# epam/ai-dial-rag

Hardware: AMD Instinct MI355X
Metric: retrieval_qps_10Mx384 (higher is better)
Workload: dtype f32 (int8 MFMA filter with exact integer dot products and a rigorous error margin, every candidate the margin cannot exclude re-scored in f64 with the reference formula)

## Files before the change

ai-dial-rag_amd/csrc/vec_index.hip:

```cpp
#include <algorithm>
#include <cmath>
#include <cstdarg>
#include <cstdio>
#include <cstdlib>
#include <cstring>
#include <mutex>
#include <new>
#include <type_traits>
#include <vector>

#include "common.h"
#include "vec_kernels.h"
#include "vec_kernels_f16.h"
#include "vec_kernels_q16.h"
#include "vec_kernels_h16.h"
#include "vec_kernels_sieve.h"
#include "vec_kernels_i8.h"
#include "vec_kernels_exact.h"
#include "vec_kernels_scoped.h"

namespace mir {

static thread_local char g_err[512] = "";

// ... 174 lines not shown
static void launch_row_norms(const T *src, int64_t n, int d, mir_index *ix, hipStream_t stream) {
    unsigned int *mx = reinterpret_cast<unsigned int *>(ix->d_maxnorm);
    const int rows_per_wg = std::min<int64_t>(128, kNormsLdsBytes / ((int64_t)norms_row_stride(d) * 4));
    if (rows_per_wg >= 32) {
        const size_t lds = (size_t)rows_per_wg * norms_row_stride(d) * 4;
        row_norms_lds_kernel<T><<<dim3((unsigned)((n + rows_per_wg - 1) / rows_per_wg)), dim3(256), lds, stream>>>(
            src, n, d, rows_per_wg, ix->d_docsq, ix->d_invnorm, mx);
    } else {
        row_norms_kernel<T><<<dim3((unsigned)((n + 255) / 256)), dim3(256), 0, stream>>>(src, n, d, ix->d_docsq, ix->d_invnorm, mx);
    }
}

static int32_t build_derived(mir_index *ix, hipStream_t stream) {
    const int64_t n = ix->n;
    const int d = ix->d;
    ix->ksteps = ix->native16 ? (d + 511) / 512 * 32 : pad_ksteps(d);
    ix->layout16 = !ix->native16 && (ix->ksteps == 8 || ix->ksteps == 16 || ix->ksteps == 24);
    ix->n_tiles = (uint32_t)((n + kTileRows - 1) / kTileRows);
    ix->hi_only = ix->layout16 && sieve_sized(ix);
    ix->wide16 = wide64_split(ix) && sieve_sized(ix);
    ix->ks16 = ix->wide16 ? (d + 511) / 512 * 32 : 0;
    const size_t split_bytes = ix->wide16 ? 16 : (size_t)ix->n_tiles * ix->ksteps * ((ix->native16 || ix->hi_only) ? 1024 : 2048);
    const size_t aux_bytes = (size_t)(ix->n_tiles + 1) * kTileRows * sizeof(float);
    MIR_HIP(hipMalloc(&ix->d_split, std::max<size_t>(split_bytes, 16)));
    MIR_HIP(hipMalloc(&ix->d_docsq, std::max<size_t>(aux_bytes, 16)));
    MIR_HIP(hipMalloc(&ix->d_invnorm, std::max<size_t>(aux_bytes, 16)));
    MIR_HIP(hipMalloc(&ix->d_maxnorm, 32));
    MIR_HIP(hipMalloc(&ix->d_dnorm, std::max<size_t>((size_t)n * 4, 16)));
    ix->hbm_bytes += split_bytes + 2 * aux_bytes + 32 + (size_t)n * 4;
    MIR_HIP(hipMemsetAsync(ix->d_docsq, 0, std::max<size_t>(aux_bytes, 16), stream));
    MIR_HIP(hipMemsetAsync(ix->d_invnorm, 0, std::max<size_t>(aux_bytes, 16), stream));
    MIR_HIP(hipMemsetAsync(ix->d_maxnorm, 0, 32, stream));
    MIR_HIP(hipMemsetAsync(reinterpret_cast<char *>(ix->d_maxnorm) + 16, 0xff, 4, stream));
    MIR_HIP(hipMalloc(reinterpret_cast<void **>(&ix->d_stats), 64));
    MIR_HIP(hipMemsetAsync(ix->d_stats, 0, 64, stream));
    if (n > 0) {
        const int64_t total_lanes = (int64_t)ix->n_tiles * ix->ksteps * 64;
        const int64_t blocks = (total_lanes + 255) / 256;
        MIR_REQUIRE(blocks < (int64_t)0x7fffffff, "index too large for one pack launch");
        if (ix->native16) {
            pack_f16_16_kernel<<<dim3((unsigned)blocks), dim3(256), 0, stream>>>(ix->d_f16, n, d, ix->ksteps / 2, total_lanes,
                                                                               ix->d_split);
            MIR_HIP(hipGetLastError());
            launch_row_norms(ix->d_f16, n, d, ix, stream);
        } else if (ix->layout16) {
            const int64_t lanes16 = total_lanes;
            pack_split16_f32_kernel<<<dim3((unsigned)((lanes16 + 255) / 256)), dim3(256), 0, stream>>>(ix->d_orig, n, d, ix->ksteps / 2,
                                                                                                   lanes16, ix->d_split, ix->hi_only);
            MIR_HIP(hipGetLastError());
            launch_row_norms(ix->d_orig, n, d, ix, stream);
        } else if (ix->wide16) {
            const int64_t lanes = (int64_t)ix->n_tiles * ix->ks16 * 64;
            MIR_HIP(hipMalloc(reinterpret_cast<void **>(&ix->d_hi16), (size_t)ix->n_tiles * ix->ks16 * 1024));
            ix->hbm_bytes += (size_t)ix->n_tiles * ix->ks16 * 1024;
            pack_hi16_f32_kernel<<<dim3((unsigned)((lanes + 255) / 256)), dim3(256), 0, stream>>>(ix->d_orig, n, d, ix->ks16 / 2, lanes, ix->d_hi16);
            MIR_HIP(hipGetLastError());
            launch_row_norms(ix->d_orig, n, d, ix, stream);
        } else {
            pack_split_f32_kernel<<<dim3((unsigned)blocks), dim3(256), 0, stream>>>(ix->d_orig, n, d, ix->ksteps,
                                                                                  total_lanes, ix->d_split);
            MIR_HIP(hipGetLastError());
            launch_row_norms(ix->d_orig, n, d, ix, stream);
        }
        MIR_HIP(hipGetLastError());
        if (ix->native16) row_dnorm_kernel<_Float16><<<dim3((unsigned)((n + 3) / 4)), dim3(256), 0, stream>>>(ix->d_f16, n, d, ix->d_dnorm);
        else row_dnorm_kernel<float><<<dim3((unsigned)((n + 3) / 4)), dim3(256), 0, stream>>>(ix->d_orig, n, d, ix->d_dnorm);
        MIR_HIP(hipGetLastError());
        if (ix->layout16) {
// ... 350 lines not shown

template <int KIND>
static int32_t launch_sieve(const mir_index *ix, int qpw, const uint4 *qsplit_g, const double *q_norm_g, const double *q_sq_g,
                            const double *q_err_g, int nq, int nwg,
                            uint32_t tile0, uint32_t n_tiles, int nan_guard, const uint64_t *gthr_g, uint64_t *cand, float *candv,
                            uint32_t *ccount, float *part_sample, bool sample, unsigned long long *stat, hipStream_t stream) {
    const float *aux = scan_aux<KIND>(ix);
    const int ks32 = ix->ksteps / 2;
    const size_t lds = sieve_lds_bytes(ks32);
    const uint32_t n_rows = (uint32_t)ix->n;
#define MIR_SIEVE_PICK(KS, P)                                                                                          \
    (qpw > 128 ? (sample ? sieve_q16_kernel<KS, KIND, true, 2, P> : sieve_q16_kernel<KS, KIND, false, 2, P>)           \
               : (sample ? sieve_q16_kernel<KS, KIND, true, 1, P> : sieve_q16_kernel<KS, KIND, false, 1, P>))
    auto go = [&](auto kern) {
        return launch_dyn(kern, dim3(nwg), dim3(512), lds, stream, ix->d_split, aux, qsplit_g, q_norm_g, q_sq_g, q_err_g, ix->d_maxnorm,
                          n_rows, tile0, n_tiles, nq, nan_guard, gthr_g, cand, candv, ccount, part_sample, stat,
                          (uint32_t)(ks32 * 2 * 64), ix->d_tilemax);
    };
    switch (ks32) {
        case 4: return go(ix->norms_spread ? MIR_SIEVE_PICK(4, true) : MIR_SIEVE_PICK(4, false));
        case 8: return go(ix->norms_spread ? MIR_SIEVE_PICK(8, true) : MIR_SIEVE_PICK(8, false));
        case 12: return go(ix->norms_spread ? MIR_SIEVE_PICK(12, true) : MIR_SIEVE_PICK(12, false));
        default:
            set_error("internal: the sieve has no instance for %d k-steps of 32", ks32);
            return MIR_ERR_UNSUPPORTED;
    }
#undef MIR_SIEVE_PICK
}

template <int KIND>
static int32_t launch_sieve_i8(const mir_index *ix, int qpw, const float *q_scale_g, const uint4 *qfrag_g, const double *q_norm_g,
                               const double *q_sq_g, const double *q_err_g, int nq, int nwg, uint32_t stage0, uint32_t n_stages,
                               int nan_guard, const uint64_t *gthr_g, uint64_t *cand, float *candv, uint32_t *ccount, float *part_sample,
                               bool sample, unsigned long long *stat, hipStream_t stream) {
    const bool four = nq >= kI8FourWaveQueries;
    const size_t lds = sieve_i8_lds_bytes(ix->ks64, four ? 4 : 8);
    const uint32_t n_rows = (uint32_t)ix->n;
    const int grid = (four && !sample) ? 2 * nwg : nwg;
#define MIR_I8_PICK(KS)                                                                                                \
    (four ? (qpw > 128 ? (sample ? sieve_i8_kernel<KS, KIND, true, 4, 4> : sieve_i8_kernel<KS, KIND, false, 4, 4>)     \
                       : (sample ? sieve_i8_kernel<KS, KIND, true, 2, 4> : sieve_i8_kernel<KS, KIND, false, 2, 4>))    \
          : (qpw > 128 ? (sample ? sieve_i8_kernel<KS, KIND, true, 2, 8> : sieve_i8_kernel<KS, KIND, false, 2, 8>)     \
                       : (sample ? sieve_i8_kernel<KS, KIND, true, 1, 8> : sieve_i8_kernel<KS, KIND, false, 1, 8>)))
    auto go = [&](auto kern) {
        return launch_dyn(kern, dim3(grid), dim3(four ? 256 : 512), lds, stream, ix->d_i8,
                          ix->d_i8rec + (KIND == SCAN_COS ? (size_t)ix->n_stages * 72 : 0), qfrag_g, q_norm_g, q_sq_g, q_err_g, ix->d_i8stats,
                          q_scale_g, n_rows, stage0, n_stages, nq, nan_guard, gthr_g, cand, candv, ccount, part_sample, stat);
    };
    switch (ix->ks64) {
        case 2: return go(MIR_I8_PICK(2));
        case 4: return go(MIR_I8_PICK(4));
        case 6: return go(MIR_I8_PICK(6));
        default:
            set_error("internal: the int8 filter has no instance for %d k-steps of 64", ix->ks64);
            return MIR_ERR_UNSUPPORTED;
    }
#undef MIR_I8_PICK
}

template <int KIND, bool BF = false>
static int32_t launch_sieve16(const mir_index *ix, const uint4 *qfrag_g, const float *qscale_g, const double *q_norm_g, const double *q_sq_g,
                              int nq, int nwg, uint32_t tile0, uint32_t n_tiles, int nan_guard, const uint64_t *gthr_g, uint64_t *cand,
                              float *candv, uint32_t *ccount, float *part_sample, bool sample, unsigned long long *stat, hipStream_t stream,
                              const double *q_err_g = nullptr) {
    const float *aux = scan_aux<KIND>(ix);
    const size_t lds = sieve16_lds_bytes();
    const uint32_t n_rows = (uint32_t)ix->n;
    const uint4 *image = BF ? ix->d_hi16 : ix->d_split;
    const int ks = BF ? ix->ks16 : ix->ksteps;
    auto go = [&](auto kern) {
        return launch_dyn(kern, dim3(nwg), dim3(512), lds, stream, image, aux, qfrag_g, qscale_g, q_norm_g, q_sq_g, q_err_g, ix->d_maxnorm,
                          n_rows, tile0, n_tiles, nq, nan_guard, gthr_g, cand, candv, ccount, part_sample, stat);
    };
    if (ks == 64) return go(sample ? sieve_h16_kernel<32, KIND, true, BF> : sieve_h16_kernel<32, KIND, false, BF>);
    if (ks == 32) return go(sample ? sieve_h16_kernel<16, KIND, true, BF> : sieve_h16_kernel<16, KIND, false, BF>);
    set_error("internal: the float16 sieve has no instance for %d k-steps", ks);
    return MIR_ERR_UNSUPPORTED;
}

template <int KIND>
// ... 170 lines not shown
    } else if (ix->native16) {
        const int ks32 = ix->ksteps / 2, ntiles16 = ngroups * (kQ16Queries / 16);
        query_stats_h16_kernel<<<dim3(std::max(b, (gwords + 63) / 64)), dim3(64), 0, stream>>>(dq, b, d, sb.q_sq, sb.q_norm, sb.qscale, gz, gwords);
        prep_queries_h16_kernel<<<dim3(ntiles16 * ks32), dim3(64), 0, stream>>>(dq, b, d, ks32, sb.qscale, sb.qsplit);
    } else {
        const int ntiles32 = ngroups * (qpw / 32);
        const int prep_blocks = std::max(ntiles32 * ix->ksteps + b, (gwords + 63) / 64);
        prep_queries_kernel<<<dim3(prep_blocks), dim3(64), 0, stream>>>(dq, b, d, ix->ksteps, ntiles32, sb.qsplit, sb.q_sq, sb.q_norm, gz, gwords);
    }
    MIR_HIP(hipGetLastError());
    return MIR_OK;
}

struct SieveGroup {
    int g, q0, nq;
    int guard;
    uint64_t *gthr;
};

static int32_t sieve_filter(const SearchCall &c, const SieveGroup &sg, uint32_t t0, uint32_t nt, int wgs, uint64_t *cand, float *cv,
                            uint32_t *cc, bool smp) {
    mir_index *ix = c.ix;
    const SearchBuffers &sb = c.sb;
    const hipStream_t stream = c.stream;
    const int g = sg.g, q0 = sg.q0, nq = sg.nq, guard = sg.guard, qpw = c.pl.qpw;
    uint64_t *gt = sg.gthr;
    const double *qn = sb.q_norm + q0, *qsq = sb.q_sq + q0, *qerr = sb.q_err + q0;
    float *ps = reinterpret_cast<float *>(sb.part_sample);
    unsigned long long *st = smp ? nullptr : ix->d_stats + (t0 ? 1 : 0);
    if (c.use_i8) {
        const uint32_t s0 = t0 / 2, s1 = std::min<uint32_t>((t0 + nt + 1) / 2, ix->n_stages);
        const uint4 *qf = sb.qsplit + (size_t)g * (qpw / 16) * ix->ks64 * 64;
        return with_kind(c.metric, [&](auto kind) {
            return launch_sieve_i8<kind()>(ix, qpw, sb.qscale + q0, qf, qn, qsq, qerr, nq, wgs, s0, s1 - s0, guard, gt, cand, cv, cc, ps, smp, st, stream);
        });
    }
    if (ix->native16) {
        const uint4 *qs16 = sb.qsplit + (size_t)g * (kQ16Queries / 16) * (ix->ksteps / 2) * 64;
        const float *qsc = sb.qscale + (size_t)g * qpw;
        return with_kind(c.metric, [&](auto kind) {
            return launch_sieve16<kind()>(ix, qs16, qsc, qn, qsq, nq, wgs, t0, nt, guard, gt, cand, cv, cc, ps, smp, st, stream);
        });
    }
    if (ix->wide16) {
        const uint4 *qw = sb.qsplit + (size_t)g * (kQ16Queries / 16) * (ix->ks16 / 2) * 128;
        return with_kind(c.metric, [&](auto kind) {
            return launch_sieve16<kind(), true>(ix, qw, nullptr, qn, qsq, nq, wgs, t0, nt, guard, gt, cand, cv, cc, ps, smp, st, stream, qerr);
        });
    }
    const uint4 *qs = sb.qsplit + (size_t)g * (qpw / 32) * ix->ksteps * 128;
    return with_kind(c.metric, [&](auto kind) {
        return launch_sieve<kind()>(ix, qpw, qs, qn, qsq, qerr, nq, wgs, t0, nt, guard, gt, cand, cv, cc, ps, smp, st, stream);
    });
}

static SieveSelectArgs sieve_select_args(const SearchCall &c, const SieveGroup &sg) {
    const mir_index *ix = c.ix;
    const SearchBuffers &sb = c.sb;
    SieveSelectArgs sa;
    sa.l = sb.sv; sa.q0 = sg.q0; sa.nq = sg.nq; sa.k = c.k; sa.metric = c.metric; sa.d = ix->d; sa.nan_guard = sg.guard;
    sa.rel_err = ix->native16 ? (float)kH16RelErr : kHiHiRelErr;
    sa.extra_slop = ix->wide16 ? wide_accum_slop(ix->ks16 * 16) : 0.f;
    sa.docs = ix->d_orig; sa.docs16 = ix->d_f16; sa.doc_sq = ix->d_docsq;
    sa.dnorm = (ix->native16 || !ix->norms_spread) ? nullptr : ix->d_dnorm;
    sa.q = c.dq; sa.q_sq = sb.q_sq; sa.q_norm = sb.q_norm; sa.max_norm = ix->d_maxnorm;
    sa.q_err = ix->native16 ? nullptr : sb.q_err;
    sa.i8_qscale = nullptr;
// ... 21 lines not shown
    sg.g = g; sg.q0 = qpw * g; sg.nq = std::min(qpw, c.b - qpw * g);
    sg.guard = c.metric == MIR_METRIC_EUCLIDEAN_DIST ? 1 : 0;
    sg.gthr = sb.gthr + (size_t)g * std::max(128, qpw);
    const int nq = sg.nq;
    unsigned long long *gt = reinterpret_cast<unsigned long long *>(sg.gthr);
    SieveScatterArgs ca;
    ca.q0 = sg.q0; ca.nq = nq; ca.l = sb.sv;
    SieveSelectArgs sa = sieve_select_args(c, sg);
    int32_t rc = sieve_filter(c, sg, 0, (uint32_t)kSampleWgs * pl.sample_tpw, kSampleWgs, nullptr, nullptr, nullptr, true);
    if (rc != MIR_OK) return rc;
    if (c.use_i8) {
        SieveSampleArgs ta;
        ta.part = reinterpret_cast<const float *>(sb.part_sample); ta.nwg = kSampleWgs; ta.qpw = qpw; ta.k = k; ta.nq = nq;
        ta.q0 = sg.q0; ta.d = ix->d; ta.metric = c.metric; ta.docs = ix->d_orig; ta.doc_sq = ix->d_docsq;
        ta.q = c.dq; ta.q_sq = sb.q_sq; ta.q_norm = sb.q_norm; ta.gthr = gt;
        sieve_sample_threshold_kernel<<<dim3(nq), dim3(256), 0, stream>>>(ta);
    } else {
        sample_threshold_kernel<<<dim3(nq), dim3(256), 0, stream>>>(reinterpret_cast<const float *>(sb.part_sample), kSampleWgs, qpw, k, nq, gt);
    }
    MIR_HIP(hipGetLastError());
    ProfileBracket prof(ix, stream);
    rc = prof.begin();
    if (rc != MIR_OK) return rc;
    for (int phase = pl.tiles_first ? 0 : 1; phase < 2; ++phase) {
        const size_t region = c.use_i8 ? (size_t)kI8Region : (size_t)kSieveRegion;
        uint64_t *cand = sb.sv_cand + (size_t)phase * nwg * region;
        float *cv = sb.sv_candv + (size_t)phase * nwg * region;
        uint32_t *cc = sb.sv_ccount + (size_t)phase * nwg * (c.use_i8 ? 8 : 1);
        rc = phase == 0 ? sieve_filter(c, sg, 0, pl.tiles_first, nwg, cand, cv, cc, false)
                        : sieve_filter(c, sg, pl.tiles_first, ix->n_tiles - pl.tiles_first, nwg, cand, cv, cc, false);
        if (rc == MIR_OK && phase == 1) rc = prof.end();
        if (rc != MIR_OK) return rc;
        ca.cand = cand; ca.candv = cv; ca.ccount = cc;
        if (c.use_i8) sieve_scatter_i8_kernel<<<dim3(nwg * 8), dim3(256), 0, stream>>>(ca);
        else sieve_scatter_kernel<<<dim3(nwg * kSieveScatterSplit), dim3(256), 0, stream>>>(ca);
        sa.mode = phase;
        rc = launch_dyn(sieve_select_kernel, dim3(nq), dim3(kSieveSelectThreads), sieve_select_lds_bytes(), stream, sa);
        if (rc != MIR_OK) return rc;
    }
    return MIR_OK;
}

static int32_t enqueue_list_group(const SearchCall &c, int g) {
    const mir_index *ix = c.ix;
    const SearchBuffers &sb = c.sb;
    const hipStream_t stream = c.stream;
    const int nwg = c.pl.nwg, klist = c.pl.klist, qpw = c.pl.qpw, metric = c.metric;
    const uint4 *qs = sb.qsplit + (size_t)g * (qpw / 32) * ix->ksteps * 128;
    uint64_t *pg = sb.part + (size_t)g * nwg * qpw * klist;
    const int nq = std::min(qpw, c.b - qpw * g);
    ProfileBracket prof(c.ix, stream);
    int32_t rc = prof.begin();
    if (rc != MIR_OK) return rc;
    if (qpw == 32) {
        rc = with_kind(metric, [&](auto kind) { return launch_scan<kind()>(ix, qs, nq, klist, nwg, pg, stream); });
    } else if (ix->native16) {
        const uint4 *qs16 = sb.qsplit + (size_t)g * (kQ16Queries / 16) * (ix->ksteps / 2) * 64;
        const float *qsc = sb.qscale + (size_t)g * qpw;
        rc = with_kind(metric, [&](auto kind) { return launch_scan_h16<kind()>(ix, qs16, qsc, nq, klist, nwg, pg, sb.gthr + (size_t)g * 128, stream); });
    } else if (ix->layout16) {
        const double *qn = sb.q_norm + (size_t)g * qpw;
        rc = with_kind(metric, [&](auto kind) { return launch_scan_q16<kind()>(ix, qs, qn, nq, klist, nwg, pg, stream); });
    } else {
        rc = with_kind(metric, [&](auto kind) { return launch_scan_f16<kind()>(ix, qs, nq, klist, nwg, pg, stream); });
    }
    if (rc != MIR_OK) return rc;
    return prof.end();
}
// ... 422 lines not shown
    double ms = 0.0;
    for (auto &pr : ev) {
        float t = 0.f;
        hipError_t e = hipEventSynchronize(pr.second);
        if (e == hipSuccess) e = hipEventElapsedTime(&t, pr.first, pr.second);
        {
            std::lock_guard<std::mutex> lk(idx->mu);
            idx->prof_free.push_back(pr.first);
            idx->prof_free.push_back(pr.second);
        }
        if (e != hipSuccess) {
            set_error("profile read failed: %s", hipGetErrorString(e));
            return MIR_ERR_HIP;
        }
        ms += t;
    }
    std::lock_guard<std::mutex> lk(idx->mu);
    idx->prof_launches += (int64_t)ev.size();
    idx->prof_ms += ms;
    if (launches) *launches = idx->prof_launches;
    if (total_ms) *total_ms = idx->prof_ms;
    if (reset) {
        idx->prof_launches = 0;
        idx->prof_ms = 0.0;
    }
    return MIR_OK;
}

int32_t mir_index_scan_stats(mir_index *idx, int32_t reset, int64_t *out8) {
    MIR_REQUIRE(idx != nullptr && out8 != nullptr, "NULL argument");
    int32_t rc = use_device(idx->device, nullptr);
    if (rc != MIR_OK) return rc;
    MIR_HIP(hipDeviceSynchronize());
    MIR_HIP(hipMemcpy(out8, idx->d_stats, 64, hipMemcpyDeviceToHost));
    if (reset) MIR_HIP(hipMemset(idx->d_stats, 0, 64));
    out8[6] = idx->i8 ? 1 : 0;
    return MIR_OK;
}

int32_t mir_index_search_device(mir_index *idx, const double *queries_device, int32_t b, int32_t k,
                                int32_t metric, int32_t *out_doc, int64_t *out_chunk, int64_t *out_row,
                                double *out_dist, int32_t *out_count, int32_t *out_flags, void *stream_) {
    int32_t rc = check_search_args(idx, queries_device, b, k, metric, out_count);
    if (rc != MIR_OK) return rc;
    if (b == 0) return MIR_OK;
    rc = use_device(idx->device, nullptr);
    if (rc != MIR_OK) return rc;
    SearchPlan pl;
    rc = plan(idx, b, k, &pl);
    if (rc != MIR_OK) return rc;
    SearchBuffers sb;
    const SearchOut out{out_doc, out_chunk, out_row, out_dist, out_count, out_flags};
    return with_workspace(
        idx, static_cast<hipStream_t>(stream_), false, [&](char *base) { return carve(sb, base, idx, b, k, pl, false); },
        [&](Workspace *, hipStream_t s) { return enqueue_search(idx, queries_device, b, k, metric, sb, pl, out, s); });
}

int32_t mir_index_search(mir_index *idx, const double *queries_host, int32_t b, int32_t k, int32_t metric,
                         int32_t *out_doc, int64_t *out_chunk, int64_t *out_row, double *out_dist,
                         int32_t *out_count, int32_t *out_flags) {
    int32_t rc = check_search_args(idx, queries_host, b, k, metric, out_count);
    if (rc != MIR_OK) return rc;
    if (b == 0) return MIR_OK;
    rc = use_device(idx->device, nullptr);
    if (rc != MIR_OK) return rc;
    SearchPlan pl;
    rc = plan(idx, b, k, &pl);
    if (rc != MIR_OK) return rc;
// ... 409 lines not shown
```

ai-dial-rag_amd/csrc/vec_kernels_i8.h:

```cpp
#pragma once
#include "vec_kernels_sieve.h"

#ifndef I8_ABL
#define I8_ABL 0
#endif

namespace mir {

typedef int __attribute__((ext_vector_type(4))) i32x4;

constexpr int kI8StatWords = 8;
constexpr int kI8MaxK = 16;
static_assert(kI8MaxK <= kSieveSampleMaxK, "the exact sample threshold evaluates k rows in one round");
constexpr int kI8Region = 32768;
constexpr int kI8WavePart = kI8Region / 8;
__device__ __forceinline__ void i8_margin_ab(float qn, float eq, const float *__restrict__ stats, float &A, float &B) {
    i8_margin_ab_decl(qn, eq, stats, A, B);
}
__device__ __forceinline__ float i8_margin_tile(bool l2, float A, float B, float e_t, float s_t, float sq) {
    const float m = fmaf(e_t, A, B) + 2.0f * s_t * sq;
    return l2 ? 2.0f * m : m;
}

__global__ __launch_bounds__(256) void i8_tile_scale_kernel(const float *__restrict__ src, int64_t n, int d, float4 *__restrict__ tparam) {
// ... 137 lines not shown
        qfrag[(int64_t)blk * 64 + lane] = make_uint4(wv[0], wv[1], wv[2], wv[3]);
    } else {
        const int qi = blk - ntiles16 * ks64;
        if (qi >= b) return;
        const float m = q_amax[qi];
        const bool ok = m >= 0.f;
        const float inv = m > 0.f ? 127.0f / m : 1.0f;
        const float sq = 1.0f / inv;
        double e2 = 0.0;
        for (int j = lane; j < d; j += 64) {
            const double x = q[(int64_t)qi * d + j];
            const double r = ok ? x - (double)sq * (double)i8_quant((float)x, inv) : x;
            e2 += r * r;
        }
        e2 = wave_sum(e2);
        if (lane == 0) {
            q_err[qi] = sqrt(e2);
            q_scale[qi] = sq;
        }
    }
}

__host__ __device__ constexpr int sieve_i8_stages(int nw) { return nw == 8 ? kSieveStages : 3; }
__host__ __device__ constexpr size_t sieve_i8_lds_bytes(int ks64, int nw) { return (size_t)sieve_i8_stages(nw) * (ks64 * 4 * 1024 + (64 + 8) * 4) + 64; }

template <int KS64, int KIND, bool SAMPLE, int QT, int NW>
__global__ __launch_bounds__(NW * 64, 2) void sieve_i8_kernel(const uint4 *__restrict__ docs, const float *__restrict__ aux,
                                                          const uint4 *__restrict__ qfrag, const double *__restrict__ q_norm,
                                                          const double *__restrict__ q_sq, const double *__restrict__ q_err,
                                                          const float *__restrict__ stats, const float *__restrict__ q_scale,
                                                          uint32_t n_rows, uint32_t stage0, uint32_t n_stages, int nq, int nan_guard,
                                                          const uint64_t *__restrict__ gthr, uint64_t *__restrict__ cand,
                                                          float *__restrict__ candv, uint32_t *__restrict__ ccount,
                                                          float *__restrict__ part_sample, unsigned long long *__restrict__ stat) {
    static_assert(KIND == SCAN_L2 || KIND == SCAN_IP || KIND == SCAN_COS, "scan kind");
    static_assert(QT == 1 || QT == 2 || QT == 4, "query tiles per wave");
    static_assert(NW == 8 || NW == 4, "waves per workgroup");
    constexpr int NS = sieve_i8_stages(NW);
    constexpr int APW = 64 / NW;
    constexpr int NB = KS64 * 2;
    constexpr int SB = NB * 2;
    constexpr int STAGE_U4 = SB * 64;
    constexpr int PPW = SB / NW;
    constexpr int PW = PPW + 1;
    constexpr int AS = 64 + 8;
    constexpr int D = NS - 1;
    constexpr int QPL = NW * 16 * QT;
    static_assert(SB % NW == 0, "sieve_i8: d padded to a multiple of 128");
    extern __shared__ __attribute__((aligned(16))) unsigned char smem[];
    uint4 *ring = reinterpret_cast<uint4 *>(smem);
    float *aux_lds = reinterpret_cast<float *>(smem + (size_t)NS * STAGE_U4 * 16);

    const int tid = threadIdx.x, lane = tid & 63, qc = lane & 15, jg = lane >> 4;
    const int wave8 = __builtin_amdgcn_readfirstlane(tid >> 6);
    const uint32_t G = gridDim.x;

    const float amin = KIND == SCAN_L2 ? stats[7] : 0.f;
    int qloc[QT];
    bool lane_live[QT];
    unsigned long long live_mask[QT];
    constexpr float L = KIND == SCAN_L2 ? 2.0f : 1.0f;
    const float ax_hi = KIND == SCAN_COS ? stats[6] : 1.0f;
    float tbc[QT];
    float sq[QT], mA[QT], mB[QT], P1[QT], A1[QT], guard[QT], best[QT];
    uint32_t brow[QT];
    i32x4 qh[QT][KS64];
    const bool active = nq > wave8 * QT * 16;
// ... 189 lines not shown
            if (KS64 < QT + 1 && have_prev) {
#pragma unroll
                for (int u = KS64 - 1; u < QT; ++u) filter(u, p0[u], p1[u], pax, pt, ptp);
            }
#pragma unroll
            for (int u = 0; u < QT; ++u) { p0[u] = c0[u]; p1[u] = c1[u]; }
#pragma unroll
            for (int i = 0; i < 8; ++i) pax[i] = cax[i];
            ptp = ctp;
            pt = stage * 2 + sub;
            have_prev = true;
        }
    }
    if (have_prev) {
#pragma unroll
        for (int u = 0; u < QT; ++u) filter(u, p0[u], p1[u], pax, pt, ptp);
    }
    if (SAMPLE) {
        uint32_t *part_row = reinterpret_cast<uint32_t *>(part_sample + (size_t)gridDim.x * QPL * 2);
#pragma unroll
        for (int u = 0; u < QT; ++u) {
            const float o = __shfl_xor(best[u], 16, 64);
            const uint32_t orow = (uint32_t)__shfl_xor((int)brow[u], 16, 64);
            const bool other = o > best[u];
            const float b2 = other ? o : best[u];
            const size_t at = ((size_t)blockIdx.x * QPL + qloc[u]) * 2 + (jg >> 1);
            if (lane_live[u] && (jg == 0 || jg == 2)) {
                part_sample[at] = b2;
                part_row[at] = other ? orow : brow[u];
            }
        }
        return;
    }
    if (lane == 0) {
        ccount[(size_t)blockIdx.x * NW + wave8] = wcount;
        if (stat && wcount) atomicAdd(stat, (unsigned long long)wcount);
    }
}

__global__ __launch_bounds__(256) void sieve_scatter_i8_kernel(SieveScatterArgs a) {
    __shared__ uint32_t s_cnt[256], s_base[256];
    const int tid = threadIdx.x;
    const int part = blockIdx.x;
    uint32_t cnt = a.ccount[part];
    s_cnt[tid] = 0;
    __syncthreads();
    if (cnt > (uint32_t)kI8WavePart) {
        for (int i = tid; i < a.nq; i += 256) a.l.over[a.q0 + i] = 1;
        cnt = kI8WavePart;
    }
    const uint64_t *region = a.cand + (size_t)part * kI8WavePart;
    const float *regionv = a.candv + (size_t)part * kI8WavePart;
    for (uint32_t e = tid; e < cnt; e += 256) atomicAdd(&s_cnt[(int)(region[e] >> 32) & 255], 1u);
    __syncthreads();
    {
        const uint32_t c = s_cnt[tid];
        s_base[tid] = c ? atomicAdd(&a.l.count[(size_t)(a.q0 + tid) * kSieveCountStride], c) : 0u;
        s_cnt[tid] = 0;
    }
    __syncthreads();
    for (uint32_t e = tid; e < cnt; e += 256) {
        const uint64_t key = region[e];
        const int ql = (int)(key >> 32) & 255, qi = a.q0 + ql;
        const uint32_t slot = s_base[ql] + atomicAdd(&s_cnt[ql], 1u);
        if (slot < (uint32_t)kSieveQueryCap) {
            a.l.row[(size_t)qi * kSieveQueryCap + slot] = (uint32_t)key;
            a.l.rv[(size_t)qi * kSieveQueryCap + slot] = regionv[e];
        } else {
            a.l.over[qi] = 1;
        }
    }
}

}
```

ai-dial-rag_amd/csrc/vec_kernels_sieve.h:

```cpp
#pragma once
#include "vec_kernels_q16.h"
#include "vec_kernels_h16.h"

#ifndef SIEVE_ABL
#define SIEVE_ABL 0
#endif
#ifndef SIEVE_MAX3
#define SIEVE_MAX3 1
#endif
#ifndef SIEVE_SELECT_ABL
#define SIEVE_SELECT_ABL 0
#endif
#ifndef SIEVE_PREFETCH
#define SIEVE_PREFETCH 2
#endif

namespace mir {

constexpr int kSieveStages = 6;
#ifndef MIR_SIEVE_REGION
#define MIR_SIEVE_REGION 8192
#endif
constexpr int kSieveRegion = MIR_SIEVE_REGION;
constexpr int kSieveQueryCap = 16384;
constexpr int kSieveSelectCap = 4096;
constexpr int kSieveMaxK = 64;
constexpr int kSieveCountStride = 32;

constexpr int kSieveAuxStride = kTileRows + 8;
__host__ __device__ constexpr size_t sieve_lds_bytes(int ks32) { return (size_t)kSieveStages * (ks32 * 2 * 1024 + kSieveAuxStride * 4) + 64; }

template <int KS32, int KIND, bool SAMPLE, int QT, bool PTMT>
__global__ __launch_bounds__(512, 2) void sieve_q16_kernel(const uint4 *__restrict__ docs, const float *__restrict__ aux,
                                                           const uint4 *__restrict__ qsplit, const double *__restrict__ q_norm,
                                                           const double *__restrict__ q_sq, const double *__restrict__ q_err,
                                                           const float *__restrict__ max_norm,
                                                           uint32_t n_rows, uint32_t tile0, uint32_t n_tiles, int nq, int nan_guard,
                                                           const uint64_t *__restrict__ gthr, uint64_t *__restrict__ cand,
                                                           float *__restrict__ candv, uint32_t *__restrict__ ccount,
                                                           float *__restrict__ part_sample, unsigned long long *__restrict__ stat,
                                                           uint32_t tile_u4,
                                                           const float *__restrict__ tile_max) {
    static_assert(QT == 1 || QT == 2, "query tiles per wave");
    constexpr int NS = kSieveStages;
    constexpr int SB = KS32 * 2;
    constexpr int STAGE_U4 = SB * 64;
    constexpr int PPW = SB / 8;
    constexpr bool AUX = KIND != SCAN_IP;
    constexpr bool PTM = PTMT && KIND != SCAN_COS;
    constexpr int PW = PPW + ((AUX || PTM) ? 1 : 0);
    constexpr int AS = kSieveAuxStride;
    constexpr int D = NS - 1;
    constexpr int QPL = 128 * QT;
    static_assert(SB % 8 == 0, "sieve: d padded to a multiple of 128");
    extern __shared__ __attribute__((aligned(16))) unsigned char smem[];
    uint4 *ring = reinterpret_cast<uint4 *>(smem);
    float *aux_lds = reinterpret_cast<float *>(smem + (size_t)NS * STAGE_U4 * 16);
    uint32_t *s_count = reinterpret_cast<uint32_t *>(aux_lds + NS * AS);

    const int tid = threadIdx.x, lane = tid & 63, qc = lane & 15, jg = lane >> 4;
// ... 230 lines not shown
#pragma unroll
            for (int u = 0; u < QT; ++u)
                if (s == 2 + u && have_prev) {
                    __builtin_amdgcn_sched_barrier(0);
#if SIEVE_ABL != 4
                    filter(u, p0[u], p1[u], pax, pt, p_tmax);
#else
                    if (g == 0xffffff) filter(u, p0[u], p1[u], pax, pt, p_tmax);
#endif
                }
        }
#pragma unroll
        for (int u = 0; u < QT; ++u) { p0[u] = c0[u]; p1[u] = c1[u]; }
        pt = t; have_prev = true; p_tmax = c_tmax;
#pragma unroll
        for (int i = 0; i < 8; ++i) pax[i] = cax[i];
    }
    if (have_prev) {
#pragma unroll
        for (int u = 0; u < QT; ++u) filter(u, p0[u], p1[u], pax, pt, p_tmax);
    }
    if (SAMPLE) {
#pragma unroll
        for (int u = 0; u < QT; ++u) {
            const float o = __shfl_xor(best[u], 16, 64);
            const float b2 = fmaxf(best[u], o);
            if (lane_live[u] && (jg == 0 || jg == 2)) part_sample[((size_t)blockIdx.x * QPL + qloc[u]) * 2 + (jg >> 1)] = b2;
        }
        return;
    }
    __syncthreads();
    if (tid == 0) {
        ccount[blockIdx.x] = *s_count;
        if (stat && *s_count) atomicAdd(stat, (unsigned long long)*s_count);
    }
}

constexpr int kSieve16Stages = 4;
__host__ __device__ constexpr size_t sieve16_lds_bytes() { return (size_t)kSieve16Stages * (kH16StageKs * 2048 + kTileRows * 4) + 64; }

template <int KS32, int KIND, bool SAMPLE, bool BF = false>
__global__ __launch_bounds__(512, 2) void sieve_h16_kernel(const uint4 *__restrict__ docs, const float *__restrict__ aux,
                                                           const uint4 *__restrict__ qfrag, const float *__restrict__ qscale_inv,
                                                           const double *__restrict__ q_norm, const double *__restrict__ q_sq,
                                                           const double *__restrict__ q_err,
                                                           const float *__restrict__ max_norm, uint32_t n_rows, uint32_t tile0,
                                                           uint32_t n_tiles, int nq, int nan_guard, const uint64_t *__restrict__ gthr,
                                                           uint64_t *__restrict__ cand, float *__restrict__ candv,
                                                           uint32_t *__restrict__ ccount, float *__restrict__ part_sample,
                                                           unsigned long long *__restrict__ stat) {
    static_assert(KS32 % kH16StageKs == 0, "float16 sieve: d padded to a multiple of 512");
    constexpr int NS = kSieve16Stages;
    constexpr int SPT = KS32 / kH16StageKs;
    constexpr int SB = kH16StageKs * 2;
    constexpr int STAGE_U4 = SB * 64;
    constexpr int TILE_U4 = SPT * STAGE_U4;
    constexpr int PPW = SB / 8;
    constexpr bool AUX = KIND != SCAN_IP;
    constexpr int PW = PPW + (AUX ? 1 : 0);
    constexpr int D = NS - 1;
    extern __shared__ __attribute__((aligned(16))) unsigned char smem[];
    uint4 *ring = reinterpret_cast<uint4 *>(smem);
    float *aux_lds = reinterpret_cast<float *>(smem + (size_t)NS * STAGE_U4 * 16);
    uint32_t *s_count = reinterpret_cast<uint32_t *>(aux_lds + NS * kTileRows);

    const int tid = threadIdx.x, lane = tid & 63, qc = lane & 15, jg = lane >> 4;
    const int wave8 = __builtin_amdgcn_readfirstlane(tid >> 6);
// ... 139 lines not shown
                if (BF) {
                    c0 = __builtin_amdgcn_mfma_f32_16x16x32_bf16(__builtin_bit_cast(bf16x8, f0[s % 3]), __builtin_bit_cast(bf16x8, qh[j * kH16StageKs + s]), c0, 0, 0, 0);
                    c1 = __builtin_amdgcn_mfma_f32_16x16x32_bf16(__builtin_bit_cast(bf16x8, f1[s % 3]), __builtin_bit_cast(bf16x8, qh[j * kH16StageKs + s]), c1, 0, 0, 0);
                } else {
                    c0 = __builtin_amdgcn_mfma_f32_16x16x32_f16(__builtin_bit_cast(f16x8, f0[s % 3]), __builtin_bit_cast(f16x8, qh[j * kH16StageKs + s]), c0, 0, 0, 0);
                    c1 = __builtin_amdgcn_mfma_f32_16x16x32_f16(__builtin_bit_cast(f16x8, f1[s % 3]), __builtin_bit_cast(f16x8, qh[j * kH16StageKs + s]), c1, 0, 0, 0);
                }
                if (s == 1) {
                    __builtin_amdgcn_sched_barrier(0);
                    if (g + D < NG) issue(g + D);
                }
                if (j == 0 && s == 2 && have_prev) {
                    __builtin_amdgcn_sched_barrier(0);
                    filter(p0, p1, pax, pt);
                }
            }
        }
        if (active) {
            p0 = c0; p1 = c1; pt = t; have_prev = true;
#pragma unroll
            for (int i = 0; i < 8; ++i) pax[i] = cax[i];
        }
    }
    if (have_prev) filter(p0, p1, pax, pt);
    if (SAMPLE) {
        const float o = __shfl_xor(best, 16, 64);
        const float b2 = fmaxf(best, o);
        if (lane_live && (jg == 0 || jg == 2)) part_sample[((size_t)blockIdx.x * kQ16Queries + qloc) * 2 + (jg >> 1)] = b2;
        return;
    }
    __syncthreads();
    if (tid == 0) {
        ccount[blockIdx.x] = *s_count;
        if (stat && *s_count) atomicAdd(stat, (unsigned long long)*s_count);
    }
}

struct SieveLists {
    float *rv;
    uint32_t *row;
    uint32_t *count;
    uint32_t *over;
};

struct SieveScatterArgs {
    const uint64_t *cand;
    const float *candv;
    const uint32_t *ccount;
    int q0, nq;
    SieveLists l;
};

constexpr int kSieveScatterSplit = 2;
__global__ __launch_bounds__(256) void sieve_scatter_kernel(SieveScatterArgs a) {
    const int tid = threadIdx.x;
    const int reg = blockIdx.x / kSieveScatterSplit, part = blockIdx.x % kSieveScatterSplit;
    uint32_t cnt = a.ccount[reg];
    if (cnt > (uint32_t)kSieveRegion) {
        if (part == 0)
            for (int i = tid; i < a.nq; i += 256) a.l.over[a.q0 + i] = 1;
        cnt = kSieveRegion;
    }
    const uint64_t *region = a.cand + (size_t)reg * kSieveRegion;
    const float *regionv = a.candv + (size_t)reg * kSieveRegion;
    for (uint32_t e = part * 256 + tid; e < cnt; e += 256 * kSieveScatterSplit) {
        const uint64_t key = region[e];
        const float v = regionv[e];
// ... 174 lines not shown
    int32_t *flagged;
    unsigned long long *stats;
    double *qt;
};

__host__ __device__ constexpr size_t sieve_select_lds_bytes() {
    return (size_t)kSieveQueryCap * 4 + 16 + (size_t)kSieveSelectCap * 18 + 16 * 64 * 4;
}
constexpr int kSieveSelectThreads = 1024;
__global__ __launch_bounds__(kSieveSelectThreads) void sieve_select_kernel(SieveSelectArgs a) {
    extern __shared__ __attribute__((aligned(16))) unsigned char sel_lds[];
    constexpr size_t kOffD = (size_t)kSieveQueryCap * 4 + 16;
    float *s_v = reinterpret_cast<float *>(sel_lds);
    double *s_d = reinterpret_cast<double *>(sel_lds + kOffD);
    float *s_x = reinterpret_cast<float *>(sel_lds + kOffD + (size_t)kSieveSelectCap * 8);
    uint32_t *s_row = reinterpret_cast<uint32_t *>(sel_lds + kOffD + (size_t)kSieveSelectCap * 12);
    uint16_t *s_fin = reinterpret_cast<uint16_t *>(sel_lds + kOffD + (size_t)kSieveSelectCap * 16);
    uint32_t *part = reinterpret_cast<uint32_t *>(sel_lds + kOffD + (size_t)kSieveSelectCap * 18);
    __shared__ int s_ns, s_f, s_f1, s_slot, s_have, s_nn;
    __shared__ float s_kv;
    constexpr int NT = kSieveSelectThreads;
    const int tid = threadIdx.x, lane = tid & 63, wave = tid >> 6;
    const int qi = a.q0 + blockIdx.x;
    const uint32_t total = a.l.count[(size_t)qi * kSieveCountStride];
    const int n = (int)(total < (uint32_t)kSieveQueryCap ? total : (uint32_t)kSieveQueryCap);
    const uint32_t *lr = a.l.row + (size_t)qi * kSieveQueryCap;
    const float *lv = a.l.rv + (size_t)qi * kSieveQueryCap;
    const bool over = a.l.over[qi] != 0;
    if (tid == 0) { s_ns = 0; s_f = 0; s_f1 = 0; s_have = 0; s_nn = 0; }
    __syncthreads();
    auto to_exact_pass = [&]() {
        if (a.mode != 1) return;
        if (tid == 0) {
            atomicAdd(a.stats + 3, 1ull);
            s_slot = atomicAdd(a.nflag, 1);
            a.flagged[s_slot] = qi;
            if (a.out_flags) a.out_flags[qi] = MIR_FLAG_EXACT_PASS;
            if (a.out_count) a.out_count[qi] = 0;
        }
        __syncthreads();
        exact_publish_query(a.qt, s_slot, a.q + (size_t)qi * a.d, a.d, a.metric, a.q_norm[qi], tid, NT);
    };
    const bool served = query_filterable(!(a.metric == MIR_METRIC_INNER_PRODUCT || a.metric == MIR_METRIC_COSINE_SIM), a.q_norm[qi],
                                         a.max_norm[0]);
    if (over || !served) {
        to_exact_pass();
        return;
    }
    auto kth_largest = [&](const float *vals, int m) -> float {
        __syncthreads();
        if (m <= NT) sieve_wave_topk<1>(vals, m, a.k, tid, NT, part + wave * 64);
        else if (m <= 2 * NT) sieve_wave_topk<2>(vals, m, a.k, tid, NT, part + wave * 64);
        else if (m <= 4 * NT) sieve_wave_topk<4>(vals, m, a.k, tid, NT, part + wave * 64);
        else sieve_wave_topk<kSieveQueryCap / kSieveSelectThreads>(vals, m, a.k, tid, NT, part + wave * 64);
        __syncthreads();
        if (wave == 0) {
            const int nw = m <= NT ? (m + 63) / 64 : NT / 64;
            uint32_t r[16];
#pragma unroll
            for (int j = 0; j < 16; ++j) {
                const int i = j * 64 + lane;
                r[j] = i < nw * a.k ? part[(i / a.k) * 64 + i % a.k] : 0u;
            }
            uint32_t wm = 0;
            for (int t = 0; t < a.k; ++t) wm = sieve_extract_max<16>(r, lane);
            if (lane == 0) s_kv = unorderable(wm);
        }
// ... 89 lines not shown
                s_x[i] = dist == dist ? (float)rv : -__builtin_inff();
            }
        }
        __syncthreads();
    };
    auto count_numeric = [&](int m) {
        for (int i0 = 0; i0 < m; i0 += NT) {
            const int i = i0 + tid;
            const bool num = i < m && s_x[i] > -__builtin_inff();
            const unsigned long long bal = __ballot(num);
            if (bal && lane == __builtin_ctzll(bal)) atomicAdd(&s_nn, __popcll(bal));
        }
        __syncthreads();
    };
    if (a.mode == 0) {
        if (have) {
            float thr = kv - 4e-6f * fabsf(kv) - eps_m;
            compact(1, &s_f);
            const int f1 = s_f;
            if (f1 <= kSieveSelectCap) {
                evaluate(0, f1);
                count_numeric(f1);
                if (s_nn >= a.k) {
                    const float rk = kth_largest(s_x, f1);
                    const float need = rk - 4e-6f * fabsf(rk) - eps_m;
                    thr = need > thr ? need : thr;
                }
            }
            if (tid == 0) {
                const unsigned long long key = (unsigned long long)orderable(thr) << 32;
                if (thr == thr && key > a.gthr[blockIdx.x]) a.gthr[blockIdx.x] = key;
            }
        }
        if (tid == 0) atomicAdd(a.stats + 4, (unsigned long long)n);
        return;
    }
    compact(1, &s_f);
    const int f1 = s_f;
    if (tid == 0) s_f1 = f1;
    compact(2, &s_f);
    int f = s_f;
    if (f > kSieveSelectCap) {
        to_exact_pass();
        return;
    }
#if SIEVE_SELECT_ABL == 1
    return;
#endif
    const bool two_rounds = f - f1 > 128;
    evaluate(0, two_rounds ? f1 : f);
#if SIEVE_SELECT_ABL == 2
    return;
#endif
    if (two_rounds) {
        count_numeric(f1);
        if (s_nn >= a.k) {
            const float rk = kth_largest(s_x, f1);
            const float need = rk - 4e-6f * fabsf(rk) - eps_m;
            if (tid == 0) s_f = f1;
            __syncthreads();
            for (int i0 = f1; i0 < f; i0 += NT) {
                const int i = i0 + tid;
                uint16_t e = 0;
                uint32_t er = 0;
                bool keep = false;
                if (i < f) {
                    e = s_fin[i];
// ... 23 lines not shown
            }
        }
        if (tid == 0) s_nn = 0;
        __syncthreads();
        for (int i0 = 0; i0 < f; i0 += NT) {
            const int i = i0 + tid;
            const bool num = i < f && s_x[i] > -__builtin_inff();
            const unsigned long long bal = __ballot(num);
            if (bal && lane == __builtin_ctzll(bal)) atomicAdd(&s_nn, __popcll(bal));
        }
        __syncthreads();
        pre = s_nn >= a.k;
    }
    const float kx = pre ? kth_largest(s_x, f) : -__builtin_inff();
    const int kout = a.k < f ? a.k : f;
    for (int i = tid; i < f; i += NT) {
        if (pre && s_x[i] < kx) continue;
        const double dd = s_d[i];
        const uint32_t rr = s_row[i];
        int rank = 0;
        for (int c = 0; c < f; ++c) {
            if (pre && s_x[c] < kx) continue;
            rank += dist_before(s_d[c], s_row[c], dd, rr) ? 1 : 0;
        }
        if (rank < a.k) {
            const size_t o = (size_t)qi * a.k + rank;
            if (a.out_row) a.out_row[o] = a.row_offset + (int64_t)rr;
            if (a.out_dist) a.out_dist[o] = dd;
            if (a.out_doc) a.out_doc[o] = a.doc_ids ? a.doc_ids[rr] : 0;
            if (a.out_chunk) a.out_chunk[o] = a.chunk_ids ? a.chunk_ids[rr] : (int64_t)rr;
        }
    }
    if (tid == 0) {
        atomicAdd(a.stats + 5, (unsigned long long)f);
        atomicAdd(a.stats + 2, 1ull);
        if (a.out_count) a.out_count[qi] = kout;
        if (a.out_flags) a.out_flags[qi] = 0;
    }
}

constexpr int kSieveSampleMaxK = 16;
struct SieveSampleArgs {
    const float *part;
    int nwg, qpw, k, nq, q0, d, metric;
    const float *docs, *doc_sq;
    const double *q, *q_sq, *q_norm;
    unsigned long long *gthr;
};
__global__ __launch_bounds__(256) void sieve_sample_threshold_kernel(SieveSampleArgs a) {
    constexpr int kMaxVals = 2 * 256;
    __shared__ unsigned long long keys[kMaxVals];
    __shared__ float s_x[kSieveSampleMaxK];
    const int tid = threadIdx.x, lane = tid & 63, wave = tid >> 6;
    const int q = blockIdx.x;
    if (q >= a.nq || a.k > kSieveSampleMaxK) return;
    const uint32_t *prow = reinterpret_cast<const uint32_t *>(a.part + (size_t)a.nwg * a.qpw * 2);
    const int n = 2 * a.nwg;
    for (int e = tid; e < kMaxVals; e += 256) {
        unsigned long long key = 0;
        if (e < n) {
            const size_t at = ((size_t)(e >> 1) * a.qpw + q) * 2 + (e & 1);
            const float v = a.part[at];
            if (v > -__builtin_inff()) key = ((unsigned long long)orderable(v) << 32) | prow[at];
        }
        keys[e] = key;
    }
    for (int size = 2; size <= kMaxVals; size <<= 1)
        for (int stride = size >> 1; stride > 0; stride >>= 1) {
// ... 43 lines not shown
```

Baseline: 250,700.

## Shard sieve stat counters and group several i8 scatter parts per block

Global statistics atomics now go to 128 strided shards instead of one word, which is meant to cut contention on a single hot address. The host sums the shards when it reads stats. The int8 candidate count atomic moves out of the filter kernel into the scatter kernel. The scatter kernel now handles several wave parts per 256-thread block, so fewer, fuller blocks run when per-wave counts are small. In exchange each part gets fewer threads for its histogram and scatter loops, and the stats buffer is larger.

```diff
diff --git a/ai-dial-rag_amd/csrc/vec_index.hip b/ai-dial-rag_amd/csrc/vec_index.hip
--- a/ai-dial-rag_amd/csrc/vec_index.hip
+++ b/ai-dial-rag_amd/csrc/vec_index.hip
@@ -230,8 +230,8 @@
     MIR_HIP(hipMemsetAsync(ix->d_invnorm, 0, std::max<size_t>(aux_bytes, 16), stream));
     MIR_HIP(hipMemsetAsync(ix->d_maxnorm, 0, 32, stream));
     MIR_HIP(hipMemsetAsync(reinterpret_cast<char *>(ix->d_maxnorm) + 16, 0xff, 4, stream));
-    MIR_HIP(hipMalloc(reinterpret_cast<void **>(&ix->d_stats), 64));
-    MIR_HIP(hipMemsetAsync(ix->d_stats, 0, 64, stream));
+    MIR_HIP(hipMalloc(reinterpret_cast<void **>(&ix->d_stats), kSieveStatBytes));
+    MIR_HIP(hipMemsetAsync(ix->d_stats, 0, kSieveStatBytes, stream));
     if (n > 0) {
         const int64_t total_lanes = (int64_t)ix->n_tiles * ix->ksteps * 64;
         const int64_t blocks = (total_lanes + 255) / 256;
@@ -648,7 +648,7 @@
 static int32_t launch_sieve_i8(const mir_index *ix, int qpw, const float *q_scale_g, const uint4 *qfrag_g, const double *q_norm_g,
                                const double *q_sq_g, const double *q_err_g, int nq, int nwg, uint32_t stage0, uint32_t n_stages,
                                int nan_guard, const uint64_t *gthr_g, uint64_t *cand, float *candv, uint32_t *ccount, float *part_sample,
-                               bool sample, unsigned long long *stat, hipStream_t stream) {
+                               bool sample, hipStream_t stream) {
     const bool four = nq >= kI8FourWaveQueries;
     const size_t lds = sieve_i8_lds_bytes(ix->ks64, four ? 4 : 8);
     const uint32_t n_rows = (uint32_t)ix->n;
@@ -661,7 +661,7 @@
     auto go = [&](auto kern) {
         return launch_dyn(kern, dim3(grid), dim3(four ? 256 : 512), lds, stream, ix->d_i8,
                           ix->d_i8rec + (KIND == SCAN_COS ? (size_t)ix->n_stages * 72 : 0), qfrag_g, q_norm_g, q_sq_g, q_err_g, ix->d_i8stats,
-                          q_scale_g, n_rows, stage0, n_stages, nq, nan_guard, gthr_g, cand, candv, ccount, part_sample, stat);
+                          q_scale_g, n_rows, stage0, n_stages, nq, nan_guard, gthr_g, cand, candv, ccount, part_sample);
     };
     switch (ix->ks64) {
         case 2: return go(MIR_I8_PICK(2));
@@ -898,7 +898,7 @@
         const uint32_t s0 = t0 / 2, s1 = std::min<uint32_t>((t0 + nt + 1) / 2, ix->n_stages);
         const uint4 *qf = sb.qsplit + (size_t)g * (qpw / 16) * ix->ks64 * 64;
         return with_kind(c.metric, [&](auto kind) {
-            return launch_sieve_i8<kind()>(ix, qpw, sb.qscale + q0, qf, qn, qsq, qerr, nq, wgs, s0, s1 - s0, guard, gt, cand, cv, cc, ps, smp, st, stream);
+            return launch_sieve_i8<kind()>(ix, qpw, sb.qscale + q0, qf, qn, qsq, qerr, nq, wgs, s0, s1 - s0, guard, gt, cand, cv, cc, ps, smp, stream);
         });
     }
     if (ix->native16) {
@@ -986,8 +986,13 @@
         if (rc == MIR_OK && phase == 1) rc = prof.end();
         if (rc != MIR_OK) return rc;
         ca.cand = cand; ca.candv = cv; ca.ccount = cc;
-        if (c.use_i8) sieve_scatter_i8_kernel<<<dim3(nwg * 8), dim3(256), 0, stream>>>(ca);
-        else sieve_scatter_kernel<<<dim3(nwg * kSieveScatterSplit), dim3(256), 0, stream>>>(ca);
+        if (c.use_i8) {
+            const int nw = nq >= kI8FourWaveQueries ? 4 : 8, n_wgs = nwg * 8 / nw;
+            unsigned long long *st = ix->d_stats + (phase && pl.tiles_first ? 1 : 0);
+            sieve_scatter_i8_kernel<<<dim3(sieve_scatter_i8_blocks(n_wgs, nw)), dim3(256), 0, stream>>>(ca, nw, n_wgs, st);
+        } else {
+            sieve_scatter_kernel<<<dim3(nwg * kSieveScatterSplit), dim3(256), 0, stream>>>(ca);
+        }
         sa.mode = phase;
         rc = launch_dyn(sieve_select_kernel, dim3(nq), dim3(kSieveSelectThreads), sieve_select_lds_bytes(), stream, sa);
         if (rc != MIR_OK) return rc;
@@ -1476,8 +1481,14 @@
     int32_t rc = use_device(idx->device, nullptr);
     if (rc != MIR_OK) return rc;
     MIR_HIP(hipDeviceSynchronize());
-    MIR_HIP(hipMemcpy(out8, idx->d_stats, 64, hipMemcpyDeviceToHost));
-    if (reset) MIR_HIP(hipMemset(idx->d_stats, 0, 64));
+    std::vector<unsigned long long> shards((size_t)kSieveStatShards * kSieveStatStride);
+    MIR_HIP(hipMemcpy(shards.data(), idx->d_stats, kSieveStatBytes, hipMemcpyDeviceToHost));
+    if (reset) MIR_HIP(hipMemset(idx->d_stats, 0, kSieveStatBytes));
+    for (int w = 0; w < 8; ++w) {
+        unsigned long long total = 0;
+        for (int s = 0; s < kSieveStatShards; ++s) total += shards[(size_t)s * kSieveStatStride + w];
+        out8[w] = (int64_t)total;
+    }
     out8[6] = idx->i8 ? 1 : 0;
     return MIR_OK;
 }
diff --git a/ai-dial-rag_amd/csrc/vec_kernels_i8.h b/ai-dial-rag_amd/csrc/vec_kernels_i8.h
--- a/ai-dial-rag_amd/csrc/vec_kernels_i8.h
+++ b/ai-dial-rag_amd/csrc/vec_kernels_i8.h
@@ -193,7 +193,7 @@
                                                           uint32_t n_rows, uint32_t stage0, uint32_t n_stages, int nq, int nan_guard,
                                                           const uint64_t *__restrict__ gthr, uint64_t *__restrict__ cand,
                                                           float *__restrict__ candv, uint32_t *__restrict__ ccount,
-                                                          float *__restrict__ part_sample, unsigned long long *__restrict__ stat) {
+                                                          float *__restrict__ part_sample) {
     static_assert(KIND == SCAN_L2 || KIND == SCAN_IP || KIND == SCAN_COS, "scan kind");
     static_assert(QT == 1 || QT == 2 || QT == 4, "query tiles per wave");
     static_assert(NW == 8 || NW == 4, "waves per workgroup");
@@ -449,26 +449,38 @@
         }
         return;
     }
-    if (lane == 0) {
-        ccount[(size_t)blockIdx.x * NW + wave8] = wcount;
-        if (stat && wcount) atomicAdd(stat, (unsigned long long)wcount);
-    }
-}
-
-__global__ __launch_bounds__(256) void sieve_scatter_i8_kernel(SieveScatterArgs a) {
-    __shared__ uint32_t s_cnt[256], s_base[256];
-    const int tid = threadIdx.x;
-    const int part = blockIdx.x;
-    uint32_t cnt = a.ccount[part];
+    if (lane == 0) ccount[(size_t)blockIdx.x * NW + wave8] = wcount;
+}
+
+#ifndef MIR_I8_SCATTER_GROUP
+#define MIR_I8_SCATTER_GROUP 4
+#endif
+constexpr int kI8ScatterGroup = MIR_I8_SCATTER_GROUP;
+static_assert(kI8ScatterGroup >= 1 && 256 % kI8ScatterGroup == 0, "threads per part");
+__host__ __device__ constexpr int sieve_scatter_i8_blocks(int n_wgs, int nw) { return (n_wgs + kI8ScatterGroup - 1) / kI8ScatterGroup * nw; }
+__global__ __launch_bounds__(256) void sieve_scatter_i8_kernel(SieveScatterArgs a, int nw, int n_wgs, unsigned long long *stat) {
+    constexpr int G = kI8ScatterGroup, TPP = 256 / G;
+    __shared__ uint32_t s_cnt[256], s_base[256], s_raw[G];
+    const int tid = threadIdx.x, sub = tid / TPP, lt = tid % TPP;
+    const int wg = (int)(blockIdx.x / nw) * G + sub, wave = (int)(blockIdx.x % nw);
+    const size_t part = (size_t)wg * nw + wave;
+    const uint32_t raw = wg < n_wgs ? a.ccount[part] : 0u;
+    const bool lost = raw > (uint32_t)kI8WavePart;
+    const uint32_t cnt = lost ? (uint32_t)kI8WavePart : raw;
     s_cnt[tid] = 0;
-    __syncthreads();
-    if (cnt > (uint32_t)kI8WavePart) {
+    if (lt == 0) s_raw[sub] = raw;
+    if (__syncthreads_or(lost)) {
         for (int i = tid; i < a.nq; i += 256) a.l.over[a.q0 + i] = 1;
-        cnt = kI8WavePart;
-    }
-    const uint64_t *region = a.cand + (size_t)part * kI8WavePart;
-    const float *regionv = a.candv + (size_t)part * kI8WavePart;
-    for (uint32_t e = tid; e < cnt; e += 256) atomicAdd(&s_cnt[(int)(region[e] >> 32) & 255], 1u);
+    }
+    if (stat && tid == 0) {
+        unsigned long long total = 0;
+#pragma unroll
+        for (int i = 0; i < G; ++i) total += s_raw[i];
+        if (total) sieve_stat_add(stat, blockIdx.x, total);
+    }
+    const uint64_t *region = a.cand + part * kI8WavePart;
+    const float *regionv = a.candv + part * kI8WavePart;
+    for (uint32_t e = lt; e < cnt; e += TPP) atomicAdd(&s_cnt[(int)(region[e] >> 32) & 255], 1u);
     __syncthreads();
     {
         const uint32_t c = s_cnt[tid];
@@ -476,7 +488,7 @@
         s_cnt[tid] = 0;
     }
     __syncthreads();
-    for (uint32_t e = tid; e < cnt; e += 256) {
+    for (uint32_t e = lt; e < cnt; e += TPP) {
         const uint64_t key = region[e];
         const int ql = (int)(key >> 32) & 255, qi = a.q0 + ql;
         const uint32_t slot = s_base[ql] + atomicAdd(&s_cnt[ql], 1u);
diff --git a/ai-dial-rag_amd/csrc/vec_kernels_sieve.h b/ai-dial-rag_amd/csrc/vec_kernels_sieve.h
--- a/ai-dial-rag_amd/csrc/vec_kernels_sieve.h
+++ b/ai-dial-rag_amd/csrc/vec_kernels_sieve.h
@@ -26,6 +26,13 @@
 constexpr int kSieveSelectCap = 4096;
 constexpr int kSieveMaxK = 64;
 constexpr int kSieveCountStride = 32;
+
+constexpr int kSieveStatShards = 128;
+constexpr int kSieveStatStride = 16;
+constexpr size_t kSieveStatBytes = (size_t)kSieveStatShards * kSieveStatStride * 8;
+__device__ __forceinline__ void sieve_stat_add(unsigned long long *word, uint32_t shard, unsigned long long v) {
+    atomicAdd(word + (size_t)(shard % (uint32_t)kSieveStatShards) * kSieveStatStride, v);
+}
 
 constexpr int kSieveAuxStride = kTileRows + 8;
 __host__ __device__ constexpr size_t sieve_lds_bytes(int ks32) { return (size_t)kSieveStages * (ks32 * 2 * 1024 + kSieveAuxStride * 4) + 64; }
@@ -322,7 +329,7 @@
     __syncthreads();
     if (tid == 0) {
         ccount[blockIdx.x] = *s_count;
-        if (stat && *s_count) atomicAdd(stat, (unsigned long long)*s_count);
+        if (stat && *s_count) sieve_stat_add(stat, blockIdx.x, (unsigned long long)*s_count);
     }
 }
 
@@ -528,7 +535,7 @@
     __syncthreads();
     if (tid == 0) {
         ccount[blockIdx.x] = *s_count;
-        if (stat && *s_count) atomicAdd(stat, (unsigned long long)*s_count);
+        if (stat && *s_count) sieve_stat_add(stat, blockIdx.x, (unsigned long long)*s_count);
     }
 }
 
@@ -769,7 +776,7 @@
     auto to_exact_pass = [&]() {
         if (a.mode != 1) return;
         if (tid == 0) {
-            atomicAdd(a.stats + 3, 1ull);
+            sieve_stat_add(a.stats + 3, blockIdx.x, 1ull);
             s_slot = atomicAdd(a.nflag, 1);
             a.flagged[s_slot] = qi;
             if (a.out_flags) a.out_flags[qi] = MIR_FLAG_EXACT_PASS;
@@ -925,7 +932,7 @@
                 if (thr == thr && key > a.gthr[blockIdx.x]) a.gthr[blockIdx.x] = key;
             }
         }
-        if (tid == 0) atomicAdd(a.stats + 4, (unsigned long long)n);
+        if (tid == 0) sieve_stat_add(a.stats + 4, blockIdx.x, (unsigned long long)n);
         return;
     }
     compact(1, &s_f);
@@ -1015,8 +1022,8 @@
         }
     }
     if (tid == 0) {
-        atomicAdd(a.stats + 5, (unsigned long long)f);
-        atomicAdd(a.stats + 2, 1ull);
+        sieve_stat_add(a.stats + 5, blockIdx.x, (unsigned long long)f);
+        sieve_stat_add(a.stats + 2, blockIdx.x, 1ull);
         if (a.out_count) a.out_count[qi] = kout;
         if (a.out_flags) a.out_flags[qi] = 0;
     }
```

New measurement: 243,200. 0.97x the previous value.
